# dist1ll/pomcpp

Hardware: NVIDIA B200
Metric: env-steps/sec (higher is better)
Workload: dtype u8/int32

## Files before the change

pomcpp_b200/csrc/pom_batch.cu:

```cuda
#include <cuda_runtime.h>
#include <cstdio>
#include <cstdlib>
#include <cstring>
#include <fstream>
#include <sched.h>
#include <string>
#include <vector>
#include <new>

#include "pom_batch.h"
#include "pom_kernels.cuh"

namespace
{

thread_local std::string g_err;

int fail(int code, const char* what, cudaError_t ce = cudaSuccess)
{
    g_err = what;
    if(ce != cudaSuccess)
    {
        g_err += ": ";
        g_err += cudaGetErrorString(ce);
    }
    return code;
}

struct DevBuf {
    void* p = nullptr;
    ~DevBuf() { if(p) cudaFree(p); }
    cudaError_t alloc(size_t bytes) { return cudaMalloc(&p, bytes); }
    template<typename T> T* as() const { return static_cast<T*>(p); }
};

#define CK(expr) do { cudaError_t ce_ = (expr); if(ce_ != cudaSuccess) return fail(POM_E_CUDA, #expr, ce_); } while(0)

constexpr uint64_t TILE_ALIGN = 256;
constexpr uint64_t XFER_CHUNK = 65536;
constexpr size_t   FLUSH_BYTES = size_t(256) << 20;

}

struct pom_batch {
    int       device = 0;
    uint64_t  n_envs = 0;
    uint64_t  n_alloc = 0;
    uint64_t  env_offset = 0;
    uint32_t  n_templates = 0;
    uint32_t  max_ticks = 0;
    int       tpb = 128;
    int       n_sms = 1;
    int       ws_nw = 20;
    uint32_t  attr_ws = 0;
    uint32_t  walk = 0;
    int       pingpong = 1;
    int       no_spec = 0;
    int       policy_pertick = 1;
    int       obs_fused = 0;
    int       step_kernel = 0;
    bool      teams = false;
    int       policy_view = -1;
    uint8_t*  recs = nullptr;
    uint8_t*  templates = nullptr;
    uint32_t* episodes = nullptr;
    unsigned long long* stats = nullptr;
    uint32_t* moves_buf = nullptr;
    uint8_t*  status_buf = nullptr;
    pom_state* aos_stage = nullptr;
    uint8_t*  st_stage = nullptr;
    uint32_t* bad_count = nullptr;
    uint32_t* fin_counter = nullptr;
    uint32_t* policy = nullptr;
    void*     flush_buf = nullptr;
    uint32_t* idx_buf = nullptr;
    uint64_t  idx_cap = 0;
    cudaEvent_t ev_expand = nullptr;
    cudaStream_t stream = nullptr;
    cudaEvent_t ev[2] = { nullptr, nullptr };
    static constexpr int MAX_CHUNKS = 16;
    cudaStream_t s_h2d = nullptr, s_d2h = nullptr, s_k2 = nullptr;
    cudaEvent_t ev_k2 = nullptr;
    cudaEvent_t ev_in[MAX_CHUNKS] = {}, ev_done[MAX_CHUNKS] = {}, ev_out = nullptr, ev_begin = nullptr;
    std::vector<int32_t> seeds;
    uint64_t  launches = 0;
    bool      forked = false;
    uint32_t  attr_done = 0;

    pomk::BatchParams params() const
    {
        pomk::BatchParams P;
        P.recs = recs; P.n_envs = n_envs; P.env_offset = env_offset; P.templates = templates;
        P.n_templates = n_templates; P.max_ticks = max_ticks;
        P.tmpl_mask = (n_templates & (n_templates - 1u)) == 0u ? n_templates - 1u : 0u; P.episodes = episodes; P.stats = stats;
        P.policy = policy; P.policy_stride = n_alloc;
        return P;
    }
};

namespace
{

int use(const pom_batch* cb, bool join = true)
{
    if(!cb) return fail(POM_E_ARG, "null handle");
    CK(cudaSetDevice(cb->device));
    pom_batch* b = const_cast<pom_batch*>(cb);
    if(join && b->forked)
    {
        CK(cudaEventRecord(b->ev_k2, b->s_k2));
        CK(cudaStreamWaitEvent(b->stream, b->ev_k2, 0));
        b->forked = false;
    }
    return POM_OK;
}

enum { ATTR_STEP = 1, ATTR_ROLLOUT = 2, ATTR_ROLLOUT_POLICY = 4, ATTR_POLICY_MOVES = 8, ATTR_EXPAND = 16, ATTR_OBS = 32, ATTR_ROLLOUT_SPEC = 64, ATTR_OBS_CROPPED = 128 };
constexpr uint32_t attr_bit(uint32_t which, bool teams, bool fog = false) { return (fog ? which << 16 : which) << (teams ? 8 : 0); }

uint32_t policy_view_bits(const pom_batch* b)
{
    return uint32_t(b->policy_view > 15 ? 15 : b->policy_view) << pomk::POLICY_VIEW_SHIFT;
}

template<typename K>
int set_smem(pom_batch* b, uint32_t which, K kernel, uint32_t bytes)
{
    if(b->attr_done & which) return POM_OK;
    CK(cudaFuncSetAttribute(kernel, cudaFuncAttributeMaxDynamicSharedMemorySize, int(bytes)));
    b->attr_done |= which;
    return POM_OK;
}

int ensure_stage(pom_batch* b)
{
    if(!b->aos_stage)
    {
        CK(cudaMalloc(&b->aos_stage, XFER_CHUNK * sizeof(pom_state)));
// ... 23 lines not shown
}

int build_templates_from_seeds(pom_batch* b, int32_t first_seed)
{
    const uint32_t n = b->n_templates;
    if(n > (1u << 24)) return fail(POM_E_ARG, "pom_batch_init: at most 2^24 templates");
    if(int64_t(first_seed) + 16 * int64_t(n) + 4096 > 0x7FFFFFFFll) return fail(POM_E_ARG, "pom_batch_init: first_seed too close to INT_MAX for this many templates");
    uint32_t ncand = uint32_t(n * 2.2) + 64;
    for(int attempt = 0; attempt < 6; attempt++, ncand *= 2)
    {
        DevBuf cand_b, dirty_b, pick_b;
        CK(cand_b.alloc(size_t(ncand) * POM_REC_BYTES));
        CK(dirty_b.alloc(ncand));
        uint8_t* cand = cand_b.as<uint8_t>(); uint8_t* dirty = dirty_b.as<uint8_t>();
        pomk::k_make_templates<<<(ncand + 63) / 64, 64, 0, b->stream>>>(cand, dirty, first_seed, ncand);
        b->launches++;
        CK(cudaGetLastError());
        std::vector<uint8_t> h(ncand);
        CK(cudaMemcpyAsync(h.data(), dirty, ncand, cudaMemcpyDeviceToHost, b->stream));
        CK(cudaStreamSynchronize(b->stream));
        std::vector<uint32_t> idx;
        for(uint32_t i = 0; i < ncand && idx.size() < n; i++) if(!h[i]) idx.push_back(i);
        if(idx.size() == n)
        {
            CK(pick_b.alloc(n * sizeof(uint32_t)));
            uint32_t* pick = pick_b.as<uint32_t>();
            CK(cudaMemcpyAsync(pick, idx.data(), n * sizeof(uint32_t), cudaMemcpyHostToDevice, b->stream));
            const uint64_t words = uint64_t(n) * POM_REC_WORDS;
            pomk::k_gather_records<<<unsigned((words + 255) / 256), 256, 0, b->stream>>>(
                reinterpret_cast<uint32_t*>(b->templates), reinterpret_cast<const uint32_t*>(cand), pick, n, 0);
            b->launches++;
            CK(cudaGetLastError());
            CK(cudaStreamSynchronize(b->stream));
            b->seeds.resize(n);
            for(uint32_t k = 0; k < n; k++) b->seeds[k] = first_seed + int32_t(idx[k]);
            return POM_OK;
        }
    }
    return fail(POM_E_ARG, "could not find enough clean seeds");
}

int pack_into(pom_batch* b, uint8_t* dst_recs, uint64_t first, uint64_t count, const pom_state* states, const uint8_t* status, uint32_t* bad_total)
{
    int rc = ensure_stage(b);
    if(rc) return rc;
    for(uint64_t done = 0; done < count; done += XFER_CHUNK)
    {
        const uint64_t c = count - done < XFER_CHUNK ? count - done : XFER_CHUNK;
        CK(cudaMemcpyAsync(b->aos_stage, states + done, c * sizeof(pom_state), cudaMemcpyHostToDevice, b->stream));
        if(status) CK(cudaMemcpyAsync(b->st_stage, status + done, c, cudaMemcpyHostToDevice, b->stream));
        CK(cudaMemsetAsync(b->bad_count, 0, sizeof(uint32_t), b->stream));
        pomk::k_pack<<<unsigned((c + 127) / 128), 128, 0, b->stream>>>(b->aos_stage, status ? b->st_stage : nullptr, dst_recs, first + done, c, b->bad_count);
        b->launches++;
        CK(cudaGetLastError());
        uint32_t bad = 0;
        CK(cudaMemcpyAsync(&bad, b->bad_count, sizeof(uint32_t), cudaMemcpyDeviceToHost, b->stream));
        CK(cudaStreamSynchronize(b->stream));
        *bad_total += bad;
    }
    return POM_OK;
}

constexpr int WS_NW = 20, WS_NBUF = 24;

template<int NW, bool OBS, bool FREEZE = false, bool SPEC = false, bool TEAMS = false>
int launch_step_ws(pom_batch* b, const pomk::BatchParams& P, const pomk::StepIO& io, uint32_t flags, cudaStream_t on)
{
    typedef pomk::RingScratch<WS_NBUF> R;
    const uint32_t bit = TEAMS ? (1u << (24 + (FREEZE ? 2 : (OBS ? 1 : 0)))) :
                         SPEC ? 2u : (FREEZE ? 1u : (1u << (NW + (OBS ? 1 : 0))));
    if(!(b->attr_ws & bit))
    {
        CK(cudaFuncSetAttribute(pomk::k_step_ws<NW, WS_NBUF, OBS, FREEZE, SPEC, TEAMS>, cudaFuncAttributeMaxDynamicSharedMemorySize, int(R::BYTES)));
        b->attr_ws |= bit;
    }
    const uint64_t n_slices = (P.n_envs + 31) / 32;
    const unsigned grid = unsigned(n_slices < uint64_t(b->n_sms) ? n_slices : uint64_t(b->n_sms));
    pomk::k_step_ws<NW, WS_NBUF, OBS, FREEZE, SPEC, TEAMS><<<grid, (NW + 1) * 32, R::BYTES, on ? on : b->stream>>>(P, io, flags);
    b->launches++;
    CK(cudaGetLastError());
    return POM_OK;
}

int launch_step_io(pom_batch* b, const pomk::BatchParams& P, pomk::StepIO io, uint32_t flags, cudaStream_t on)
{
    io.bulk = (reinterpret_cast<uintptr_t>(io.moves) & 15u) == 0u ? 1u : 0u;
    if(P.n_envs == b->n_envs && b->pingpong) io.reverse = (b->walk++) & 1u;
    if(b->teams)
    {
        if(flags & pomk::STEP_FREEZE_TRUNCATED) return launch_step_ws<WS_NW, false, true, false, true>(b, P, io, flags, on);
        if(io.obs) return launch_step_ws<WS_NW, true, false, false, true>(b, P, io, flags, on);
        return launch_step_ws<WS_NW, false, false, false, true>(b, P, io, flags, on);
    }
    if(flags & pomk::STEP_FREEZE_TRUNCATED) return launch_step_ws<WS_NW, false, true>(b, P, io, flags, on);
    if(b->ws_nw == WS_NW && (flags & ~uint32_t(POM_STEP_OVERLAP)) == uint32_t(POM_STEP_AUTORESET | POM_STEP_COUNT) && io.bulk &&
       !io.status_out && !io.obs && !io.joint && !io.done_bits && !io.fin_env && !b->no_spec)
        return launch_step_ws<WS_NW, false, false, true>(b, P, io, flags, on);
    if(io.obs) return launch_step_ws<WS_NW, true>(b, P, io, flags, on);
    switch(b->ws_nw)
    {
    case 12: return launch_step_ws<12, false>(b, P, io, flags, on);
    case 14: return launch_step_ws<14, false>(b, P, io, flags, on);
    case 16: return launch_step_ws<16, false>(b, P, io, flags, on);
    case 18: return launch_step_ws<18, false>(b, P, io, flags, on);
    case 22: return launch_step_ws<22, false>(b, P, io, flags, on);
    default: return launch_step_ws<WS_NW, false>(b, P, io, flags, on);
    }
}

template<int TPB, bool TEAMS = false>
int launch_step(pom_batch* b, const uint8_t* moves_dev, uint32_t flags, uint8_t* status_dev, uint64_t first = 0, uint64_t count = 0, cudaStream_t on = nullptr,
                bool tile_kernel = false)
{
    pomk::BatchParams P = b->params();
    if(count)
    {
        P.recs += first * POM_REC_BYTES; P.episodes += first; P.env_offset += first; P.n_envs = count;
        moves_dev += 4 * first;
        if(status_dev) status_dev += first;
    }
    if(b->step_kernel == 0 && !tile_kernel)
    {
        pomk::StepIO io{};
        io.moves = moves_dev;
        io.status_out = status_dev;
        return launch_step_io(b, P, io, flags, on);
    }
    { int rc = set_smem(b, attr_bit(ATTR_STEP, TEAMS), pomk::k_step<TPB, TEAMS>, pomk::TileScratch<TPB>::BYTES); if(rc) return rc; }
    const unsigned grid = unsigned((P.n_envs + TPB - 1) / TPB);
    pomk::k_step<TPB, TEAMS><<<grid, TPB, pomk::TileScratch<TPB>::BYTES, on ? on : b->stream>>>(P, reinterpret_cast<const uint32_t*>(moves_dev), flags, status_dev);
    b->launches++;
    CK(cudaGetLastError());
    return POM_OK;
}

template<int TPB, bool TEAMS = false, bool FOG = false>
int launch_rollout(pom_batch* b, uint32_t ticks, uint64_t seed, uint32_t tick0, uint32_t flags, const uint8_t* move_seq = nullptr)
{
    const uint32_t n_actions = (flags & POM_ROLL_HARMLESS) ? 5u : 6u, no_reset = flags & (POM_ROLL_NO_RESET | POM_ROLL_CONTINUE_UNDEFINED);
    const uint32_t mask = (flags >> POM_ROLL_SIMPLE_SHIFT) & 0xFu;
    const unsigned grid = unsigned((b->n_envs + TPB - 1) / TPB);
    if(mask)
    {
        int rc = set_smem(b, attr_bit(ATTR_ROLLOUT_POLICY, TEAMS, FOG), pomk::k_rollout<TPB, true, false, TEAMS, FOG>, pomk::TileScratch<TPB>::BYTES); if(rc) return rc;
        rc = ensure_policy(b); if(rc) return rc;
        pomk::k_rollout<TPB, true, false, TEAMS, FOG><<<grid, TPB, pomk::TileScratch<TPB>::BYTES, b->stream>>>(b->params(), ticks, seed, tick0, n_actions, no_reset,
                                                                                                     FOG ? mask | policy_view_bits(b) : mask, nullptr);
    }
    else if(!TEAMS && n_actions == 6u && no_reset == 0u && !move_seq && !b->no_spec)
    {
        int rc = set_smem(b, ATTR_ROLLOUT_SPEC, pomk::k_rollout<TPB, false, true>, pomk::TileScratch<TPB>::BYTES); if(rc) return rc;
        pomk::k_rollout<TPB, false, true><<<grid, TPB, pomk::TileScratch<TPB>::BYTES, b->stream>>>(b->params(), ticks, seed, tick0, 6u, 0u, 0u, nullptr);
    }
    else
    {
        int rc = set_smem(b, attr_bit(ATTR_ROLLOUT, TEAMS), pomk::k_rollout<TPB, false, false, TEAMS>, pomk::TileScratch<TPB>::BYTES); if(rc) return rc;
        pomk::k_rollout<TPB, false, false, TEAMS><<<grid, TPB, pomk::TileScratch<TPB>::BYTES, b->stream>>>(b->params(), ticks, seed, tick0, n_actions, no_reset, 0u, reinterpret_cast<const uint32_t*>(move_seq));
    }
    b->launches++;
    CK(cudaGetLastError());
    return POM_OK;
}

template<int TPB, bool TEAMS = false, bool FOG = false>
int launch_policy_moves(pom_batch* b, uint8_t* moves_dev, uint64_t seed, uint32_t tick, uint32_t mask, uint32_t gen_actions = 0, uint32_t freeze_truncated = 0)
{
    { int rc = set_smem(b, attr_bit(ATTR_POLICY_MOVES, TEAMS, FOG), pomk::k_policy_moves<TPB, TEAMS, FOG>, pomk::TileScratch<TPB>::BYTES); if(rc) return rc; }
    const unsigned grid = unsigned((b->n_envs + TPB - 1) / TPB);
    pomk::k_policy_moves<TPB, TEAMS, FOG><<<grid, TPB, pomk::TileScratch<TPB>::BYTES, b->stream>>>(b->params(), reinterpret_cast<uint32_t*>(moves_dev), seed, tick,
                                                                                            FOG ? mask | policy_view_bits(b) : mask, gen_actions, freeze_truncated);
    b->launches++;
    CK(cudaGetLastError());
    return POM_OK;
}

template<int TPB>
int launch_observe_planes(pom_batch* b, uint8_t* obs_dev, uint32_t mask, int view, uint32_t cropped_bytes = 0)
{
    const unsigned grid = unsigned((b->n_envs + TPB - 1) / TPB);
    const uint32_t reverse = (b->pingpong && b->walk && ((b->walk - 1u) & 1u) == 0u) ? 1u : 0u;
    if(cropped_bytes)
    {
        int rc = set_smem(b, ATTR_OBS_CROPPED, pomk::k_observe_planes<TPB, true>, pomk::TileScratch<TPB>::BYTES); if(rc) return rc;
        pomk::k_observe_planes<TPB, true><<<grid, TPB, pomk::TileScratch<TPB>::BYTES, b->stream>>>(b->params(), obs_dev, b->n_alloc, mask, view, reverse, cropped_bytes);
    }
    else
    {
        int rc = set_smem(b, ATTR_OBS, pomk::k_observe_planes<TPB, false>, pomk::TileScratch<TPB>::BYTES); if(rc) return rc;
        pomk::k_observe_planes<TPB, false><<<grid, TPB, pomk::TileScratch<TPB>::BYTES, b->stream>>>(b->params(), obs_dev, b->n_alloc, mask, view, reverse, 0u);
    }
    b->launches++;
    CK(cudaGetLastError());
    return POM_OK;
}

template<int TPB, bool TEAMS = false>
int launch_expand(pom_batch* dst, const pom_batch* src, const uint32_t* idx_dev, uint64_t n_children, uint32_t fanout, uint32_t flags)
{
    { int rc = set_smem(dst, attr_bit(ATTR_EXPAND, TEAMS), pomk::k_expand_step<TPB, TEAMS>, pomk::TileScratch<TPB>::BYTES); if(rc) return rc; }
    const unsigned grid = unsigned((n_children + TPB - 1) / TPB);
    pomk::k_expand_step<TPB, TEAMS><<<grid, TPB, pomk::TileScratch<TPB>::BYTES, dst->stream>>>(dst->recs, src->recs, idx_dev, n_children, fanout, flags);
    dst->launches++;
    CK(cudaGetLastError());
    return POM_OK;
}

}

namespace
// ... 15 lines not shown
{
bool local_cpus(int device, cpu_set_t* set)
{
    char bus[32] = {0};
    if(cudaDeviceGetPCIBusId(bus, sizeof(bus), device) != cudaSuccess) { cudaGetLastError(); return false; }
    for(char* c = bus; *c; c++) if(*c >= 'A' && *c <= 'Z') *c = char(*c - 'A' + 'a');
    std::ifstream f(std::string("/sys/bus/pci/devices/") + bus + "/local_cpulist");
    std::string list;
    if(!f || !std::getline(f, list) || list.empty()) return false;
    CPU_ZERO(set);
    int n = 0;
    size_t i = 0;
    while(i < list.size())
    {
        char* end = nullptr;
        const long lo = std::strtol(list.c_str() + i, &end, 10);
        long hi = lo;
        i = size_t(end - list.c_str());
        if(i < list.size() && list[i] == '-') { hi = std::strtol(list.c_str() + i + 1, &end, 10); i = size_t(end - list.c_str()); }
        for(long c = lo; c <= hi && c < CPU_SETSIZE; c++) { CPU_SET(int(c), set); n++; }
        if(i < list.size() && list[i] == ',') i++;
        else if(i < list.size() && (list[i] < '0' || list[i] > '9')) break;
    }
    return n > 0;
}
}

#define POM_DISPATCH(h, fn, ...) \
    do { \
        if((h)->tpb == 32) return fn<32>(__VA_ARGS__); \
        if((h)->tpb == 64) return fn<64>(__VA_ARGS__); \
        if((h)->tpb == 256) return fn<256>(__VA_ARGS__); \
        return fn<128>(__VA_ARGS__); \
    } while(0)
#define POM_DISPATCH_MODE(h, fn, ...) \
    do { \
        if((h)->teams) return fn<128, true>(__VA_ARGS__); \
        POM_DISPATCH(h, fn, __VA_ARGS__); \
    } while(0)
#define POM_DISPATCH_POLICY(h, fn, ...) \
    do { \
        if((h)->policy_view >= 0) \
        { \
            if((h)->teams) return fn<128, true, true>(__VA_ARGS__); \
            return fn<128, false, true>(__VA_ARGS__); \
        } \
        POM_DISPATCH_MODE(h, fn, __VA_ARGS__); \
    } while(0)

extern "C" {

const char* pom_last_error(void) { return g_err.c_str(); }

int pom_device_count(void)
{
    int n = 0;
    if(cudaGetDeviceCount(&n) != cudaSuccess) { cudaGetLastError(); return 0; }
    return n;
}

int pom_batch_init(pom_batch** out, int device, uint64_t n_envs, const pom_init_desc* desc)
{
    if(!out || !desc || n_envs == 0 || desc->n_templates == 0) return fail(POM_E_ARG, "pom_batch_init: bad argument");
    if(n_envs > (uint64_t(1) << 31)) return fail(POM_E_ARG, "pom_batch_init: too many envs for one handle");
    int ndev = 0;
    cudaError_t ce = cudaGetDeviceCount(&ndev);
    if(ce != cudaSuccess || ndev == 0) return fail(POM_E_CUDA, "no CUDA device: the step path has no CPU fallback", ce);
    if(device < 0 || device >= ndev) return fail(POM_E_ARG, "pom_batch_init: no such device");
    CK(cudaSetDevice(device));
    pom_batch* b = new(std::nothrow) pom_batch();
    if(!b) return fail(POM_E_NOMEM, "host allocation failed");
    b->device = device;
    b->n_envs = n_envs;
    b->n_alloc = (n_envs + TILE_ALIGN - 1) / TILE_ALIGN * TILE_ALIGN;
    b->env_offset = desc->env_offset;
    b->n_templates = desc->n_templates;
    b->max_ticks = desc->max_ticks;
    b->teams = (desc->flags & POM_INIT_TEAMS) != 0;
    cudaDeviceGetAttribute(&b->n_sms, cudaDevAttrMultiProcessorCount, device);
    if(b->n_sms < 1) b->n_sms = 1;
    if(const char* e = std::getenv("POM_STEP_KERNEL")) b->step_kernel = std::strcmp(e, "tile") == 0 ? 1 : 0;
    if(const char* e = std::getenv("POM_WS_NW")) b->ws_nw = std::atoi(e);
    if(const char* e = std::getenv("POM_STEP_PINGPONG")) b->pingpong = std::atoi(e) != 0;
    if(const char* e = std::getenv("POM_OBS_FUSED")) b->obs_fused = std::atoi(e) != 0;
    if(const char* e = std::getenv("POM_WS_NOSPEC")) b->no_spec = std::atoi(e) != 0;
    if(const char* e = std::getenv("POM_ROLL_POLICY")) b->policy_pertick = std::strcmp(e, "fused") != 0;
    if(const char* e = std::getenv("POM_TPB"))
    {
        const int t = std::atoi(e);
        if(t == 32 || t == 64 || t == 128 || t == 256) b->tpb = t;
    }
    int rc = POM_OK;
    do {
        if(cudaStreamCreateWithFlags(&b->stream, cudaStreamNonBlocking) != cudaSuccess ||
           cudaEventCreate(&b->ev[0]) != cudaSuccess || cudaEventCreate(&b->ev[1]) != cudaSuccess ||
           cudaStreamCreateWithFlags(&b->s_h2d, cudaStreamNonBlocking) != cudaSuccess ||
           cudaStreamCreateWithFlags(&b->s_d2h, cudaStreamNonBlocking) != cudaSuccess ||
           cudaStreamCreateWithFlags(&b->s_k2, cudaStreamNonBlocking) != cudaSuccess ||
           cudaEventCreateWithFlags(&b->ev_k2, cudaEventDisableTiming) != cudaSuccess ||
           cudaEventCreateWithFlags(&b->ev_out, cudaEventDisableTiming) != cudaSuccess ||
           cudaEventCreateWithFlags(&b->ev_begin, cudaEventDisableTiming) != cudaSuccess)
        { rc = fail(POM_E_CUDA, "stream/event creation failed", cudaGetLastError()); break; }
        if(cudaMalloc(&b->recs, b->n_alloc * POM_REC_BYTES) != cudaSuccess ||
           cudaMalloc(&b->templates, size_t(b->n_templates) * POM_REC_BYTES) != cudaSuccess ||
           cudaMalloc(&b->episodes, b->n_alloc * sizeof(uint32_t)) != cudaSuccess ||
           cudaMalloc(&b->stats, POM_STATS_WORDS * sizeof(unsigned long long)) != cudaSuccess ||
           cudaMalloc(&b->moves_buf, b->n_alloc * 4) != cudaSuccess ||
           cudaMalloc(&b->status_buf, b->n_alloc) != cudaSuccess)
        { rc = fail(POM_E_NOMEM, "device allocation failed", cudaGetLastError()); break; }
        if(cudaMemsetAsync(b->recs, 0, b->n_alloc * POM_REC_BYTES, b->stream) != cudaSuccess ||
           cudaMemsetAsync(b->episodes, 0, b->n_alloc * sizeof(uint32_t), b->stream) != cudaSuccess ||
           cudaMemsetAsync(b->stats, 0, POM_STATS_WORDS * sizeof(unsigned long long), b->stream) != cudaSuccess)
        { rc = fail(POM_E_CUDA, "memset failed", cudaGetLastError()); break; }
        if(desc->host_templates)
        {
            uint32_t bad = 0;
            rc = pack_into(b, b->templates, 0, b->n_templates, desc->host_templates, nullptr, &bad);
            if(rc) break;
            if(bad) { rc = fail(POM_E_STATE, "a host template cannot be represented in the packed record"); break; }
        }
        else
        {
            rc = build_templates_from_seeds(b, desc->first_seed);
            if(rc) break;
        }
        if(!(desc->flags & POM_INIT_EMPTY))
        {
            rc = fill_from_templates(b);
            if(rc) break;
        }
        if(cudaStreamSynchronize(b->stream) != cudaSuccess) { rc = fail(POM_E_CUDA, "init sync failed", cudaGetLastError()); break; }
    } while(0);
    if(rc) { pom_batch_destroy(b); return rc; }
    *out = b;
    return POM_OK;
}

int pom_batch_destroy(pom_batch* b)
{
    if(!b) return POM_OK;
    cudaSetDevice(b->device);
    if(b->s_k2) cudaStreamSynchronize(b->s_k2);
    if(b->stream) cudaStreamSynchronize(b->stream);
    cudaFree(b->recs); cudaFree(b->templates); cudaFree(b->episodes); cudaFree(b->stats);
    cudaFree(b->moves_buf); cudaFree(b->status_buf); cudaFree(b->aos_stage); cudaFree(b->st_stage);
    cudaFree(b->bad_count); cudaFree(b->flush_buf); cudaFree(b->idx_buf); if(b->ev_expand) cudaEventDestroy(b->ev_expand); cudaFree(b->policy); cudaFree(b->fin_counter);
    if(b->ev[0]) cudaEventDestroy(b->ev[0]);
    if(b->ev[1]) cudaEventDestroy(b->ev[1]);
    for(int i = 0; i < pom_batch::MAX_CHUNKS; i++) { if(b->ev_in[i]) cudaEventDestroy(b->ev_in[i]); if(b->ev_done[i]) cudaEventDestroy(b->ev_done[i]); }
    if(b->ev_out) cudaEventDestroy(b->ev_out);
    if(b->ev_begin) cudaEventDestroy(b->ev_begin);
    if(b->s_h2d) cudaStreamDestroy(b->s_h2d);
    if(b->s_d2h) cudaStreamDestroy(b->s_d2h);
    if(b->s_k2) cudaStreamDestroy(b->s_k2);
    if(b->ev_k2) cudaEventDestroy(b->ev_k2);
    if(b->stream) cudaStreamDestroy(b->stream);
    delete b;
    return POM_OK;
}

int pom_batch_sync(pom_batch* b)
{
    int rc = use(b); if(rc) return rc;
    CK(cudaStreamSynchronize(b->stream));
    return POM_OK;
}
// ... 26 lines not shown
        CK(cudaStreamSynchronize(b->stream));
    }
    return POM_OK;
}

int pom_batch_observe(pom_batch* b, uint64_t first, uint64_t count, int agent, int view, pom_state* states, uint8_t* status)
{
    int rc = use(b); if(rc) return rc;
    if(!states) return fail(POM_E_ARG, "pom_batch_observe: null output");
    if(agent < 0 || agent > 3 || view < 0) return fail(POM_E_ARG, "pom_batch_observe: agent must be 0..3 and view >= 0");
    if(first > b->n_envs || count > b->n_envs - first) return fail(POM_E_RANGE, "pom_batch_observe: range outside the batch");
    rc = ensure_stage(b); if(rc) return rc;
    for(uint64_t done = 0; done < count; done += XFER_CHUNK)
    {
        const uint64_t c = count - done < XFER_CHUNK ? count - done : XFER_CHUNK;
        pomk::k_observe<<<unsigned((c + 127) / 128), 128, 0, b->stream>>>(b->recs, b->aos_stage, b->st_stage, first + done, c, agent, view);
        b->launches++;
        CK(cudaGetLastError());
        CK(cudaMemcpyAsync(states + done, b->aos_stage, c * sizeof(pom_state), cudaMemcpyDeviceToHost, b->stream));
        if(status) CK(cudaMemcpyAsync(status + done, b->st_stage, c, cudaMemcpyDeviceToHost, b->stream));
        CK(cudaStreamSynchronize(b->stream));
    }
    return POM_OK;
}

uint64_t pom_batch_obs_stride(const pom_batch* b) { return b ? b->n_alloc : 0; }

int pom_batch_observe_planes(pom_batch* b, uint8_t* obs_dev, uint32_t agent_mask, int view)
{
    int rc = use(b); if(rc) return rc;
    if(!obs_dev) return fail(POM_E_ARG, "pom_batch_observe_planes: null output");
    if(agent_mask == 0 || agent_mask > 0xFu || view < 0) return fail(POM_E_ARG, "pom_batch_observe_planes: agent_mask must be 1..15 and view >= 0");
    POM_DISPATCH(b, launch_observe_planes, b, obs_dev, agent_mask, view);
}

int pom_device_copy(int device, void* dst, const void* src, uint64_t bytes)
{
    if(!dst || !src) return fail(POM_E_ARG, "pom_device_copy: null pointer");
    CK(cudaSetDevice(device));
    CK(cudaMemcpy(dst, src, bytes, cudaMemcpyDefault));
    return POM_OK;
}

int pom_batch_reset(pom_batch* b)
{
    int rc = use(b); if(rc) return rc;
    CK(cudaMemsetAsync(b->episodes, 0, b->n_alloc * sizeof(uint32_t), b->stream));
    CK(cudaMemsetAsync(b->stats, 0, POM_STATS_WORDS * sizeof(unsigned long long), b->stream));
    if(b->policy) CK(cudaMemsetAsync(b->policy, 0, 9 * b->n_alloc * sizeof(uint32_t), b->stream));
    return fill_from_templates(b);
}

int pom_batch_templates(pom_batch* b, pom_state* out, int32_t* seeds_out)
{
    int rc = use(b); if(rc) return rc;
    if(!out) return fail(POM_E_ARG, "pom_batch_templates: null output");
    rc = ensure_stage(b); if(rc) return rc;
    for(uint64_t done = 0; done < b->n_templates; done += XFER_CHUNK)
    {
        const uint64_t c = b->n_templates - done < XFER_CHUNK ? b->n_templates - done : XFER_CHUNK;
        pomk::k_unpack<<<unsigned((c + 127) / 128), 128, 0, b->stream>>>(b->templates, b->aos_stage, b->st_stage, done, c);
        b->launches++;
        CK(cudaGetLastError());
        CK(cudaMemcpyAsync(out + done, b->aos_stage, c * sizeof(pom_state), cudaMemcpyDeviceToHost, b->stream));
        CK(cudaStreamSynchronize(b->stream));
    }
    if(seeds_out)
    {
        for(uint32_t k = 0; k < b->n_templates; k++) seeds_out[k] = k < b->seeds.size() ? b->seeds[k] : 0;
    }
    return POM_OK;
}

int pom_batch_step(pom_batch* b, const uint8_t* moves_dev, uint32_t flags)
{
    const bool overlap = (flags & POM_STEP_OVERLAP) && b && b->n_envs >= (uint64_t(1) << 18);
    int rc = use(b, !overlap); if(rc) return rc;
    if(!moves_dev) return fail(POM_E_ARG, "pom_batch_step: null moves");
    if(!overlap) POM_DISPATCH_MODE(b, launch_step, b, moves_dev, flags, nullptr);
    static int parts = -1;
    if(parts < 0) { const char* e = std::getenv("POM_STEP_PARTS"); parts = e ? std::atoi(e) : 2; if(parts < 2 || parts > 16) parts = 2; }
    const uint64_t per = ((b->n_envs + parts - 1) / parts + 1023) / 1024 * 1024;
    const bool tile_parts = b->n_envs <= (uint64_t(1) << 19) && !b->no_spec;
    CK(cudaEventRecord(b->ev_begin, b->stream));
    CK(cudaStreamWaitEvent(b->s_k2, b->ev_begin, 0));
    int c = 0;
    for(uint64_t first = 0; first < b->n_envs; first += per, c++)
    {
        const uint64_t count = first + per <= b->n_envs ? per : b->n_envs - first;
        rc = [&]() -> int { POM_DISPATCH_MODE(b, launch_step, b, moves_dev, flags, nullptr, first, count, (c & 1) ? b->s_k2 : b->stream, tile_parts); }();
        if(rc) return rc;
    }
    b->forked = true;
    return POM_OK;
}

static int enqueue_step_pipeline(pom_batch* b, const uint8_t* moves_host, uint8_t* status_host, uint32_t flags, int chunks, uint64_t per)
{
    const uint64_t n = b->n_envs;
    CK(cudaEventRecord(b->ev_begin, b->stream));
    CK(cudaStreamWaitEvent(b->s_h2d, b->ev_begin, 0));
    if(chunks > 1) CK(cudaStreamWaitEvent(b->s_k2, b->ev_begin, 0));
    for(int c = 0; c < chunks; c++)
    {
        const uint64_t first = uint64_t(c) * per, count = (first + per <= n) ? per : n - first;
        cudaStream_t compute = (c & 1) ? b->s_k2 : b->stream;
        CK(cudaMemcpyAsync(reinterpret_cast<uint8_t*>(b->moves_buf) + 4 * first, moves_host + 4 * first, 4 * count, cudaMemcpyHostToDevice, b->s_h2d));
        CK(cudaEventRecord(b->ev_in[c], b->s_h2d));
        CK(cudaStreamWaitEvent(compute, b->ev_in[c], 0));
        const int rc = [&]() -> int { POM_DISPATCH_MODE(b, launch_step, b, reinterpret_cast<const uint8_t*>(b->moves_buf), flags,
                                                   status_host ? b->status_buf : nullptr, first, count, compute); }();
        if(rc) return rc;
        if(status_host)
        {
            CK(cudaEventRecord(b->ev_done[c], compute));
            CK(cudaStreamWaitEvent(b->s_d2h, b->ev_done[c], 0));
            CK(cudaMemcpyAsync(status_host + first, b->status_buf + first, count, cudaMemcpyDeviceToHost, b->s_d2h));
        }
    }
    if(chunks > 1)
    {
        CK(cudaEventRecord(b->ev_k2, b->s_k2));
        CK(cudaStreamWaitEvent(b->stream, b->ev_k2, 0));
    }
    if(status_host)
    {
        CK(cudaEventRecord(b->ev_out, b->s_d2h));
        CK(cudaStreamWaitEvent(b->stream, b->ev_out, 0));
    }
    return POM_OK;
}

static int launch_step_zero_copy(pom_batch* b, const uint8_t* moves_host, uint8_t* status_host, uint32_t flags)
{
    void* mdev = nullptr; void* sdev = nullptr;
    bool ok = cudaHostGetDevicePointer(&mdev, const_cast<uint8_t*>(moves_host), 0) == cudaSuccess;
    if(ok && status_host) ok = cudaHostGetDevicePointer(&sdev, status_host, 0) == cudaSuccess;
    if(!ok) { cudaGetLastError(); return 1; }
    return [&]() -> int { POM_DISPATCH_MODE(b, launch_step, b, static_cast<const uint8_t*>(mdev), flags, static_cast<uint8_t*>(sdev)); }();
}

int pom_batch_step_host_async(pom_batch* b, const uint8_t* moves_host, uint8_t* status_host, uint32_t flags)
{
    int rc = use(b); if(rc) return rc;
    if(!moves_host) return fail(POM_E_ARG, "pom_batch_step_host_async: null moves");
    rc = launch_step_zero_copy(b, moves_host, status_host, flags);
    if(rc == 1) return fail(POM_E_ARG, "pom_batch_step_host_async: the buffers must be page-locked, device-mapped memory (pom_host_alloc)");
    return rc;
}

int pom_batch_step_host(pom_batch* b, const uint8_t* moves_host, uint8_t* status_host, uint32_t flags)
{
    int rc = use(b); if(rc) return rc;
    if(!moves_host) return fail(POM_E_ARG, "pom_batch_step_host: null moves");
    const uint64_t n = b->n_envs;
    static int zerocopy = -1;
    if(zerocopy < 0) { const char* e = std::getenv("POM_ZEROCOPY"); zerocopy = e ? std::atoi(e) : 1; }
    if(zerocopy)
    {
        rc = launch_step_zero_copy(b, moves_host, status_host, flags);
        if(rc < 0) return rc;
        if(rc == 0)
        {
            CK(cudaStreamSynchronize(b->stream));
            return POM_OK;
        }
    }
    static int want = -1;
    if(want < 0) { const char* e = std::getenv("POM_CHUNKS"); want = e ? std::atoi(e) : 6; if(want < 1 || want > pom_batch::MAX_CHUNKS) want = 6; }
    int chunks = n >= (uint64_t(1) << 18) ? want : 1;
    const uint64_t per = ((n + chunks - 1) / chunks + 1023) / 1024 * 1024;
    chunks = int((n + per - 1) / per);
    for(int c = 0; c < chunks; c++)
// ... 447 lines not shown
```

pomcpp_b200/csrc/pom_kernels.cuh:

```cuda
#ifndef POM_KERNELS_CUH_
#define POM_KERNELS_CUH_

#include <cuda_runtime.h>
#include <stdint.h>
#include "pom_core.cuh"
#include "pom_policy.cuh"
#include "pom_batch.h"

namespace pomk
{

constexpr uint32_t STEP_FREEZE_TRUNCATED = 0x40000000u;

enum { ST_STEPS = 0, ST_EPISODES = 1, ST_WIN0 = 2, ST_DRAWS = 6, ST_TRUNC = 7, ST_SUMLEN = 8, ST_INVALID = 9 };

struct BatchParams {
    uint8_t*            recs;
    uint64_t            n_envs;
    uint64_t            env_offset;
    const uint8_t*      templates;
    uint32_t            n_templates;
    uint32_t            tmpl_mask;
    uint32_t            max_ticks;
    uint32_t*           episodes;
    unsigned long long* stats;
    uint32_t*           policy;
    uint64_t            policy_stride;
};

__device__ __forceinline__ uint32_t smem_u32(const void* p) { return uint32_t(__cvta_generic_to_shared(p)); }

__device__ __forceinline__ void mbar_init(uint64_t* bar, uint32_t count)
{
    asm volatile("mbarrier.init.shared::cta.b64 [%0], %1;" :: "r"(smem_u32(bar)), "r"(count));
}
__device__ __forceinline__ void fence_barrier_init()
{
    asm volatile("fence.mbarrier_init.release.cluster;" ::: "memory");
}
__device__ __forceinline__ void fence_proxy_async()
{
    asm volatile("fence.proxy.async.shared::cta;" ::: "memory");
}
__device__ __forceinline__ void mbar_expect_tx(uint64_t* bar, uint32_t bytes)
{
    asm volatile("mbarrier.arrive.expect_tx.shared::cta.b64 _, [%0], %1;" :: "r"(smem_u32(bar)), "r"(bytes) : "memory");
}
__device__ __forceinline__ void mbar_arrive(uint64_t* bar)
{
    asm volatile("mbarrier.arrive.shared::cta.b64 _, [%0];" :: "r"(smem_u32(bar)) : "memory");
}
__device__ __forceinline__ void mbar_wait(uint64_t* bar, uint32_t parity)
{
    asm volatile(
        "{\n"
        ".reg .pred p;\n"
        "WAIT_LOOP:\n"
        "mbarrier.try_wait.parity.shared::cta.b64 p, [%0], %1;\n"
        "@p bra WAIT_DONE;\n"
        "bra WAIT_LOOP;\n"
        "WAIT_DONE:\n"
        "}\n" :: "r"(smem_u32(bar)), "r"(parity) : "memory");
}
__device__ __forceinline__ void bulk_g2s(void* smem_dst, const void* gmem_src, uint32_t bytes, uint64_t* bar)
{
    asm volatile("cp.async.bulk.shared::cluster.global.mbarrier::complete_tx::bytes [%0], [%1], %2, [%3];"
                 :: "r"(smem_u32(smem_dst)), "l"(gmem_src), "r"(bytes), "r"(smem_u32(bar)) : "memory");
}
__device__ __forceinline__ void bulk_s2g(void* gmem_dst, const void* smem_src, uint32_t bytes)
{
    asm volatile("cp.async.bulk.global.shared::cta.bulk_group [%0], [%1], %2;"
                 :: "l"(gmem_dst), "r"(smem_u32(smem_src)), "r"(bytes) : "memory");
    asm volatile("cp.async.bulk.commit_group;" ::: "memory");
}
__device__ __forceinline__ void bulk_wait_read_all()
{
    asm volatile("cp.async.bulk.wait_group.read 0;" ::: "memory");
}

__device__ __forceinline__ void warp_add(unsigned long long* dst, uint32_t v)
{
    const uint32_t s = __reduce_add_sync(0xFFFFFFFFu, v);
    if((threadIdx.x & 31u) == 0u && s) atomicAdd(dst, (unsigned long long)s);
}

struct EpisodeAcc {
    uint32_t fin_draw = 0u;
    uint32_t trunc_abort = 0u;
    uint32_t win01 = 0u, win23 = 0u;
    uint32_t len = 0u;
    uint32_t steps = 0u;
    uint32_t pending = 0u;
};

__device__ __forceinline__ void acc_add(EpisodeAcc& A, bool fin, uint32_t status, uint32_t len)
{
    if(!fin) return;
    const bool done = (status & POM_STATUS_DONE) != 0u;
    const bool draw = done && (status & POM_STATUS_DRAW);
    const bool trunc = !done && (status & POM_STATUS_TRUNCATED);
    const uint32_t w = (status & POM_STATUS_WINNER_MASK) >> POM_STATUS_WINNER_SHIFT;
    A.fin_draw += 1u + (draw ? 0x10000u : 0u);
    A.trunc_abort += (trunc ? 1u : 0u) + ((!done && !trunc) ? 0x10000u : 0u);
    if(done && !draw)
    {
        const uint32_t inc = (w & 1u) ? 0x10000u : 1u;
        if(w & 2u) A.win23 += inc; else A.win01 += inc;
    }
    A.len += len;
    A.pending++;
}

__device__ __forceinline__ void acc_flush(unsigned long long* stats, EpisodeAcc& A, bool count_steps)
{
    const uint32_t lane = threadIdx.x & 31u;
    if(__reduce_or_sync(0xFFFFFFFFu, A.pending))
    {
        const uint32_t v[9] = { A.fin_draw & 0xFFFFu, A.win01 & 0xFFFFu, A.win01 >> 16, A.win23 & 0xFFFFu, A.win23 >> 16,
                                A.fin_draw >> 16, A.trunc_abort & 0xFFFFu, A.len, A.trunc_abort >> 16 };
#pragma unroll
        for(int k = 0; k < 9; k++)
        {
            const uint32_t sum = __reduce_add_sync(0xFFFFFFFFu, v[k]);
            if(lane == 0u && sum) atomicAdd(stats + 1 + k, (unsigned long long)sum);
        }
    }
    if(count_steps)
    {
        const uint32_t sum = __reduce_add_sync(0xFFFFFFFFu, A.steps);
        if(lane == 0u && sum) atomicAdd(stats + ST_STEPS, (unsigned long long)sum);
    }
    A = EpisodeAcc();
}

__device__ __forceinline__ void cp_async_4(void* smem_dst, const void* gmem_src)
{
    asm volatile("cp.async.ca.shared.global [%0], [%1], 4;" :: "r"(smem_u32(smem_dst)), "l"(gmem_src) : "memory");
}
__device__ __forceinline__ void cp_async_wait_all()
{
    asm volatile("cp.async.wait_all;" ::: "memory");
}

__device__ __forceinline__ uint32_t finish_and_reset(uint8_t* warp_recs, uint8_t* rec, const BatchParams& P, uint64_t env, bool active, bool do_reset,
                                                 uint32_t& ep_now, EpisodeAcc& acc)
{
    uint32_t st = active ? rec[R_STATUS] : 0u;
    const uint32_t len = active ? *reinterpret_cast<const uint16_t*>(rec + R_TIME) : 0u;
    if(active && !(st & POM_STATUS_DONE) && P.max_ticks && len >= P.max_ticks) st |= POM_STATUS_TRUNCATED;
    const bool fin = active && (st & (POM_STATUS_DONE | POM_STATUS_TRUNCATED | POM_STATUS_INVALID)) != 0u;
    uint32_t pending = __ballot_sync(0xFFFFFFFFu, fin);
    if(pending == 0u) return st;
    acc_add(acc, fin, st, len);
    if(!do_reset)
    {
        if(fin) rec[R_STATUS] = uint8_t(st);
        return st;
// ... 147 lines not shown
{
    const uint32_t lane = threadIdx.x & 31u, quad = lane >> 2;
    const int part = int(lane & 3u);
#pragma unroll 1
    for(uint32_t m = 0; m < 4u; m++)
    {
        const uint32_t e = quad + 8u * m;
        const bool valid = e < n_valid;
        const uint8_t* r = sslice + e * POM_REC_BYTES;
        uint8_t* out = out0 + size_t(e) * POM_OBS_BYTES;
        pomcore::ObsWindow W{};
        uint32_t lit = 0u;
        if(valid)
        {
            W = pomcore::obs_window(r, agent, view);
            lit = pomcore::observe_part_chunks(r, agent, W, out, part);
        }
        lit |= __shfl_xor_sync(FULL_WARP, lit, 1);
        lit |= __shfl_xor_sync(FULL_WARP, lit, 2);
        __syncwarp();
        if(valid) pomcore::observe_part_patches(r, W, out, part, lit);
    }
}

template<int TPB> struct TileScratch {
    static constexpr uint32_t OFF_BAR = TPB * POM_REC_BYTES;
    static constexpr uint32_t OFF_LIST = OFF_BAR + 64;
    static constexpr uint32_t BYTES = OFF_LIST + 8 * (TPB / 32);
};

template<int TPB, bool TEAMS = false>
__global__ void __launch_bounds__(TPB) k_step(BatchParams P, const uint32_t* __restrict__ moves, uint32_t flags, uint8_t* __restrict__ status_out)
{
    extern __shared__ __align__(128) uint8_t smem[];
    const uint64_t env = uint64_t(blockIdx.x) * TPB + threadIdx.x;
    const bool active = env < P.n_envs;
    const bool raw = (flags & POM_STEP_RAW) != 0u;

    constexpr uint32_t SLICE_BYTES = 32 * POM_REC_BYTES;
    const uint32_t warp = threadIdx.x >> 5, lane = threadIdx.x & 31u;
    uint64_t* bar = reinterpret_cast<uint64_t*>(smem + TileScratch<TPB>::OFF_BAR) + warp;
    uint8_t* sslice = smem + warp * SLICE_BYTES;
    uint8_t* gslice = P.recs + (size_t(blockIdx.x) * TPB + warp * 32u) * POM_REC_BYTES;
    if(lane == 0)
    {
        mbar_init(bar, 1);
        fence_barrier_init();
        mbar_expect_tx(bar, SLICE_BYTES);
        bulk_g2s(sslice, gslice, SLICE_BYTES, bar);
    }
    const uint32_t m = active ? __ldg(moves + env) : 0u;
    uint32_t ep_now = (active && (flags & POM_STEP_AUTORESET)) ? P.episodes[env] : 0u;
    __syncwarp();
    mbar_wait(bar, 0);

    uint8_t* rec = sslice + lane * POM_REC_BYTES;
    const bool stepped = active && !(rec[R_STATUS] & (raw ? POM_STATUS_INVALID : (POM_STATUS_DONE | POM_STATUS_INVALID)));
    warp_tick<TEAMS>(sslice, rec, m, stepped, raw, smem + TileScratch<TPB>::OFF_LIST + 8u * warp,
                     (flags & POM_STEP_CONTINUE_UNDEFINED) ? pomcore::F_INVALID_MASK_CONTINUE : pomcore::F_INVALID_MASK);
    EpisodeAcc acc;
    acc.steps = stepped ? 1u : 0u;
    uint32_t st_end = active ? rec[R_STATUS] : 0u;
    if(flags & POM_STEP_AUTORESET)
    {
        const uint32_t st = finish_and_reset(sslice, rec, P, env, active && stepped, true, ep_now, acc);
        if(active && stepped) st_end = st;
    }
    acc_flush(P.stats, acc, (flags & POM_STEP_COUNT) != 0u);
    if(status_out && active) status_out[env] = uint8_t(st_end);
    fence_proxy_async();
    __syncwarp();
    if(lane == 0)
    {
        bulk_s2g(gslice, sslice, SLICE_BYTES);
        bulk_wait_read_all();
    }
}

struct StepIO {
    const void* moves;
    uint32_t    joint;
    uint32_t    bulk;
    uint32_t    reverse;
    uint8_t*    status_out;
    uint32_t*   done_bits;
    uint32_t*   fin_env;
    uint8_t*    fin_status;
    uint32_t*   fin_counter;
    uint32_t*   fin_count_out;
    uint32_t    fin_capacity;
    uint8_t*    obs;
    uint64_t    obs_stride;
    uint32_t    obs_mask;
    int         obs_view;
};

__device__ __forceinline__ uint32_t moves_of_joint(uint32_t j)
{
    const uint32_t a0 = j % 6u, r1 = j / 6u, a1 = r1 % 6u, r2 = r1 / 6u, a2 = r2 % 6u, a3 = (r2 / 6u) % 6u;
    return a0 | (a1 << 8) | (a2 << 16) | (a3 << 24);
}

template<int NBUF> struct RingScratch {
    static constexpr uint32_t SLICE_BYTES = 32 * POM_REC_BYTES;
    static constexpr uint32_t SLOT = SLICE_BYTES + 128 + 16;
    static constexpr uint32_t OFF_FULL = NBUF * SLOT;
    static constexpr uint32_t MAIL = 256;
    static constexpr uint32_t OFF_MAIL = OFF_FULL + 8 * NBUF;
    static constexpr uint32_t OFF_TICKET = OFF_MAIL + 4 * MAIL;
    static constexpr uint32_t FIN_CAP = 480;
    static constexpr uint32_t OFF_FIN = OFF_TICKET + 16;
    static constexpr uint32_t OFF_FIN_ENV = OFF_FIN + 16;
    static constexpr uint32_t OFF_FIN_ST = OFF_FIN_ENV + 4 * FIN_CAP;
    static constexpr uint32_t BYTES = OFF_FIN_ST + FIN_CAP;
};

template<int NW, int NBUF, bool OBS, bool FREEZE, bool SPEC = false, bool TEAMS = false>
__global__ void __launch_bounds__((NW + 1) * 32, 1) k_step_ws(BatchParams P, StepIO io_in, uint32_t flags_in)
{
    const uint32_t flags = SPEC ? uint32_t(POM_STEP_AUTORESET | POM_STEP_COUNT) : flags_in;
    StepIO io = io_in;
    if(SPEC)
    {
        io.joint = 0u; io.bulk = 1u; io.status_out = nullptr; io.obs = nullptr; io.done_bits = nullptr; io.fin_env = nullptr;
    }
    const uint32_t* __restrict__ moves = static_cast<const uint32_t*>(io.moves);
    const uint16_t* __restrict__ joint = static_cast<const uint16_t*>(io.moves);
    uint8_t* __restrict__ status_out = io.status_out;
    const uint32_t moves_bulk = io.bulk;
    const uint32_t mv_bytes = io.joint ? 64u : 128u;
    extern __shared__ __align__(128) uint8_t smem[];
    typedef RingScratch<NBUF> R;
    uint64_t* full = reinterpret_cast<uint64_t*>(smem + R::OFF_FULL);
    volatile uint32_t* mail = reinterpret_cast<volatile uint32_t*>(smem + R::OFF_MAIL);
    uint32_t* ticket = reinterpret_cast<uint32_t*>(smem + R::OFF_TICKET);
    uint32_t* free_mask = ticket + 2;
    const uint32_t warp = threadIdx.x >> 5, lane = threadIdx.x & 31u;
    const uint64_t n_slices = (P.n_envs + 31u) / 32u;
    const uint32_t T = blockIdx.x < n_slices ? uint32_t((n_slices - blockIdx.x + gridDim.x - 1u) / gridDim.x) : 0u;
    if(threadIdx.x == 0)
    {
        for(int b = 0; b < NBUF; b++) mbar_init(full + b, 1);
        ticket[0] = 0u;
        ticket[1] = 0u;
        *free_mask = (NBUF >= 32) ? 0xFFFFFFFFu : ((1u << NBUF) - 1u);
        reinterpret_cast<uint32_t*>(smem + R::OFF_FIN)[0] = 0u;
        reinterpret_cast<uint32_t*>(smem + R::OFF_FIN)[1] = 0xFFFFFFFFu;
        fence_barrier_init();
    }
    for(uint32_t i = threadIdx.x; i < R::MAIL; i += blockDim.x) mail[i] = 0u;
    __syncthreads();

    if(warp == NW)
    {
        if(lane != 0) return;
        uint32_t parity = 0u;
        for(uint32_t t = 0; t < T; t++)
        {
            uint32_t fm;
            while((fm = *reinterpret_cast<volatile uint32_t*>(free_mask)) == 0u) __nanosleep(40);
            const uint32_t b = uint32_t(__ffs(int(fm))) - 1u;
            atomicAnd(free_mask, ~(1u << b));
            const uint64_t s0 = blockIdx.x + uint64_t(t) * gridDim.x;
            const uint64_t s = io.reverse ? n_slices - 1u - s0 : s0;
            const bool whole = (s + 1u) * 32u <= P.n_envs;
            const uint32_t mbytes = (moves_bulk && whole) ? mv_bytes : 0u;
            mbar_expect_tx(full + b, R::SLICE_BYTES + mbytes);
            bulk_g2s(smem + b * R::SLOT, P.recs + s * R::SLICE_BYTES, R::SLICE_BYTES, full + b);
            if(mbytes) bulk_g2s(smem + b * R::SLOT + R::SLICE_BYTES, static_cast<const uint8_t*>(io.moves) + s * mv_bytes, mbytes, full + b);
            mail[t % R::MAIL] = ((t + 1u) << 8) | (b << 1) | ((parity >> b) & 1u);
            parity ^= 1u << b;
        }
        return;
    }

    const bool raw = (flags & POM_STEP_RAW) != 0u;
    EpisodeAcc acc;
    for(;;)
    {
        uint32_t t = 0u;
        if(lane == 0) t = atomicAdd(ticket, 1u);
        t = __shfl_sync(FULL_WARP, t, 0);
        if(t >= T) break;
        const uint64_t s0 = blockIdx.x + uint64_t(t) * gridDim.x;
        const uint64_t s = io.reverse ? n_slices - 1u - s0 : s0;
        const uint64_t env = s * 32u + lane;
        const bool active = env < P.n_envs;
        const bool whole = (s + 1u) * 32u <= P.n_envs;
        uint32_t m = 0u;
        if(!(moves_bulk && whole) && active) m = io.joint ? uint32_t(__ldg(joint + env)) : __ldg(moves + env);
        uint32_t ep_now = (active && (flags & POM_STEP_AUTORESET)) ? P.episodes[env] : 0u;
        uint32_t v;
        while(((v = mail[t % R::MAIL]) >> 8) != t + 1u) __nanosleep(20);
        const uint32_t b = (v >> 1) & 31u;
        uint8_t* sslice = smem + b * R::SLOT;
        mbar_wait(full + b, v & 1u);
        if(moves_bulk && whole)
            m = io.joint ? uint32_t(reinterpret_cast<const uint16_t*>(sslice + R::SLICE_BYTES)[lane])
                         : reinterpret_cast<const uint32_t*>(sslice + R::SLICE_BYTES)[lane];
        if(io.joint) m = moves_of_joint(m);

        uint8_t* rec = sslice + lane * POM_REC_BYTES;
        const bool stepped = active && !(rec[R_STATUS] & ((raw ? POM_STATUS_INVALID : (POM_STATUS_DONE | POM_STATUS_INVALID)) |
                                                          (FREEZE ? POM_STATUS_TRUNCATED : 0)));
        warp_tick<TEAMS>(sslice, rec, m, stepped, raw, sslice + R::SLICE_BYTES + 128u,
                         (flags & POM_STEP_CONTINUE_UNDEFINED) ? pomcore::F_INVALID_MASK_CONTINUE : pomcore::F_INVALID_MASK);
        acc.steps += stepped ? 1u : 0u;
        uint32_t st_end = active ? rec[R_STATUS] : 0u;
        if(flags & POM_STEP_AUTORESET)
        {
            const uint32_t st = finish_and_reset(sslice, rec, P, env, active && stepped, true, ep_now, acc);
            if(active && stepped) st_end = st;
        }
        if(status_out && active) status_out[env] = uint8_t(st_end);
        if(io.done_bits || io.fin_env)
        {
            const bool ended = active && stepped && (st_end & (POM_STATUS_DONE | POM_STATUS_TRUNCATED | POM_STATUS_INVALID)) != 0u;
            const uint32_t em = __ballot_sync(FULL_WARP, ended);
            if(io.done_bits && lane == 0) io.done_bits[s] = em;
            if(io.fin_env && em)
            {
                uint32_t* fin = reinterpret_cast<uint32_t*>(smem + R::OFF_FIN);
                const uint32_t k = uint32_t(__popc(em));
                uint32_t pos = 0u;
                if(lane == 0) pos = atomicAdd(fin, k);
                pos = __shfl_sync(FULL_WARP, pos, 0);
                const uint32_t mine = uint32_t(__popc(em & ((1u << lane) - 1u)));
                if(pos + k <= R::FIN_CAP)
                {
                    if(ended)
                    {
                        reinterpret_cast<uint32_t*>(smem + R::OFF_FIN_ENV)[pos + mine] = uint32_t(env);
                        smem[R::OFF_FIN_ST + pos + mine] = uint8_t(st_end);
                    }
                }
                else
                {
                    if(lane == 0) { atomicMin(fin + 1, pos); pos = atomicAdd(io.fin_counter, k); }
                    pos = __shfl_sync(FULL_WARP, pos, 0) + mine;
                    if(ended && pos < io.fin_capacity)
                    {
                        io.fin_env[pos] = uint32_t(env);
                        io.fin_status[pos] = uint8_t(st_end);
                    }
                }
            }
        }
        fence_proxy_async();
        __syncwarp();
        if(lane == 0) bulk_s2g(P.recs + s * R::SLICE_BYTES, sslice, R::SLICE_BYTES);
        if(OBS && io.obs)
        {
            const uint32_t n_valid = whole ? 32u : uint32_t(P.n_envs - s * 32u);
            uint32_t k = 0u;
            for(int a = 0; a < 4; a++)
            {
                if(!((io.obs_mask >> a) & 1u)) continue;
                warp_observe_slice(sslice, a, io.obs_view, io.obs + (uint64_t(k) * io.obs_stride + s * 32u) * POM_OBS_BYTES, n_valid);
                k++;
            }
        }
        __syncwarp();
        if(lane == 0)
        {
            bulk_wait_read_all();
            __threadfence_block();
            atomicOr(free_mask, 1u << b);
        }
        __syncwarp();
    }
    acc_flush(P.stats, acc, (flags & POM_STEP_COUNT) != 0u);
    if(io.fin_env)
    {
        __threadfence_block();
        uint32_t* warps_done = ticket + 1;
        bool last = false;
        if(lane == 0) last = atomicAdd(warps_done, 1u) == uint32_t(NW - 1);
        last = __shfl_sync(FULL_WARP, last ? 1 : 0, 0) != 0;
        if(last)
        {
            __threadfence_block();
            const volatile uint32_t* fin = reinterpret_cast<const volatile uint32_t*>(smem + R::OFF_FIN);
            const uint32_t k = fin[1] != 0xFFFFFFFFu ? fin[1] : fin[0];
            unsigned long long old = 0ull;
            if(lane == 0) old = atomicAdd(reinterpret_cast<unsigned long long*>(io.fin_counter), (1ull << 32) | k);
            old = __shfl_sync(FULL_WARP, old, 0);
            const uint32_t base = uint32_t(old);
            for(uint32_t i = lane; i < k; i += 32u)
            {
                if(base + i < io.fin_capacity)
                {
                    io.fin_env[base + i] = reinterpret_cast<const uint32_t*>(smem + R::OFF_FIN_ENV)[i];
                    io.fin_status[base + i] = smem[R::OFF_FIN_ST + i];
                }
            }
            if(lane == 0 && uint32_t(old >> 32) == gridDim.x - 1u)
            {
                const uint32_t count = base + k;
                *io.fin_count_out = count < io.fin_capacity ? count : io.fin_capacity;
                *reinterpret_cast<volatile unsigned long long*>(io.fin_counter) = 0ull;
            }
        }
    }
}

struct GlobalAgentStore {
    uint32_t* base;
    uint64_t  stride;
    __device__ __forceinline__ pompolicy::SimpleSt load(int a) const
    {
        pompolicy::SimpleSt s;
        s.w0 = base[uint64_t(2 * a) * stride];
        s.w1 = base[uint64_t(2 * a + 1) * stride];
        return s;
    }
    __device__ __forceinline__ void store(int a, const pompolicy::SimpleSt& v)
    {
        base[uint64_t(2 * a) * stride] = v.w0;
        base[uint64_t(2 * a + 1) * stride] = v.w1;
    }
    __device__ __forceinline__ void clear(uint32_t episode)
    {
#pragma unroll
        for(int k = 0; k < 8; k++) base[uint64_t(k) * stride] = 0u;
        base[8 * stride] = episode;
    }
    __device__ __forceinline__ void claim(uint32_t episode)
    {
        if(base[8 * stride] != episode) clear(episode);
    }
};

constexpr uint32_t POLICY_VIEW_SHIFT = 8;
// ... 359 lines not shown
```

Measured before the change: 10.06 billion.

## Keep last tickets of each step part L2-resident with cache-hint bulk copies

In the split multi-stream step path, all parts now share the same walk direction, and the bulk loads and stores of env records carry L2 cache-policy hints. Earlier tickets use evict_first, and the last tickets (about 16 MB by default, set by an env var) use evict_normal. The goal is for the slices touched last by one step to still sit in L2 when the next step, walking the opposite way, reads them first, which cuts HBM traffic. It only applies when the state exceeds L2 but is at most four times L2, and it adds policy creation instructions on the producer and consumer paths.

```diff
diff --git a/pomcpp_b200/csrc/pom_batch.cu b/pomcpp_b200/csrc/pom_batch.cu
--- a/pomcpp_b200/csrc/pom_batch.cu
+++ b/pomcpp_b200/csrc/pom_batch.cu
@@ -39,6 +39,7 @@
 constexpr uint64_t TILE_ALIGN = 256;
 constexpr uint64_t XFER_CHUNK = 65536;
 constexpr size_t   FLUSH_BYTES = size_t(256) << 20;
+constexpr uint64_t L2_KEEP_MB = 16;
 
 }
 
@@ -54,6 +55,8 @@
     int       ws_nw = 20;
     uint32_t  attr_ws = 0;
     uint32_t  walk = 0;
+    uint64_t  l2_keep_bytes = uint64_t(L2_KEEP_MB) << 20;
+    uint64_t  l2_bytes = 0;
     int       pingpong = 1;
     int       no_spec = 0;
     int       policy_pertick = 1;
@@ -243,10 +246,24 @@
     return POM_OK;
 }
 
-int launch_step_io(pom_batch* b, const pomk::BatchParams& P, pomk::StepIO io, uint32_t flags, cudaStream_t on)
+uint32_t l2_keep(const pom_batch* b, uint64_t n_envs)
+{
+    if(!b->l2_keep_bytes || b->n_envs * POM_REC_BYTES <= b->l2_bytes) return 0u;
+    const uint64_t n_slices = (n_envs + 31) / 32, grid = n_slices < uint64_t(b->n_sms) ? n_slices : uint64_t(b->n_sms);
+    const uint64_t per_ticket = grid * 32 * POM_REC_BYTES, tickets = (n_slices + grid - 1) / grid;
+    const uint64_t keep = (b->l2_keep_bytes + per_ticket - 1) / per_ticket;
+    return uint32_t(keep < tickets ? keep : tickets);
+}
+
+int launch_step_io(pom_batch* b, const pomk::BatchParams& P, pomk::StepIO io, uint32_t flags, cudaStream_t on, int part = -1)
 {
     io.bulk = (reinterpret_cast<uintptr_t>(io.moves) & 15u) == 0u ? 1u : 0u;
-    if(P.n_envs == b->n_envs && b->pingpong) io.reverse = (b->walk++) & 1u;
+    if(part < 0 && P.n_envs == b->n_envs && b->pingpong) io.reverse = (b->walk++) & 1u;
+    if(part >= 0)
+    {
+        io.reverse = (b->walk - 1u) & 1u;
+        io.keep = l2_keep(b, P.n_envs);
+    }
     if(b->teams)
     {
         if(flags & pomk::STEP_FREEZE_TRUNCATED) return launch_step_ws<WS_NW, false, true, false, true>(b, P, io, flags, on);
@@ -271,7 +288,7 @@
 
 template<int TPB, bool TEAMS = false>
 int launch_step(pom_batch* b, const uint8_t* moves_dev, uint32_t flags, uint8_t* status_dev, uint64_t first = 0, uint64_t count = 0, cudaStream_t on = nullptr,
-                bool tile_kernel = false)
+                bool tile_kernel = false, int part = -1)
 {
     pomk::BatchParams P = b->params();
     if(count)
@@ -285,7 +302,7 @@
         pomk::StepIO io{};
         io.moves = moves_dev;
         io.status_out = status_dev;
-        return launch_step_io(b, P, io, flags, on);
+        return launch_step_io(b, P, io, flags, on, part);
     }
     { int rc = set_smem(b, attr_bit(ATTR_STEP, TEAMS), pomk::k_step<TPB, TEAMS>, pomk::TileScratch<TPB>::BYTES); if(rc) return rc; }
     const unsigned grid = unsigned((P.n_envs + TPB - 1) / TPB);
@@ -467,6 +484,8 @@
     if(const char* e = std::getenv("POM_STEP_KERNEL")) b->step_kernel = std::strcmp(e, "tile") == 0 ? 1 : 0;
     if(const char* e = std::getenv("POM_WS_NW")) b->ws_nw = std::atoi(e);
     if(const char* e = std::getenv("POM_STEP_PINGPONG")) b->pingpong = std::atoi(e) != 0;
+    if(const char* e = std::getenv("POM_STEP_L2_KEEP_MB")) { const uint64_t mb = std::strtoull(e, nullptr, 10); b->l2_keep_bytes = (mb < 65536 ? mb : 65536) << 20; }
+    { int l2 = 0; cudaDeviceGetAttribute(&l2, cudaDevAttrL2CacheSize, device); b->l2_bytes = uint64_t(l2 > 0 ? l2 : 0); }
     if(const char* e = std::getenv("POM_OBS_FUSED")) b->obs_fused = std::atoi(e) != 0;
     if(const char* e = std::getenv("POM_WS_NOSPEC")) b->no_spec = std::atoi(e) != 0;
     if(const char* e = std::getenv("POM_ROLL_POLICY")) b->policy_pertick = std::strcmp(e, "fused") != 0;
@@ -659,13 +678,15 @@
     if(parts < 0) { const char* e = std::getenv("POM_STEP_PARTS"); parts = e ? std::atoi(e) : 2; if(parts < 2 || parts > 16) parts = 2; }
     const uint64_t per = ((b->n_envs + parts - 1) / parts + 1023) / 1024 * 1024;
     const bool tile_parts = b->n_envs <= (uint64_t(1) << 19) && !b->no_spec;
+    const bool part_walk = !tile_parts && b->pingpong && b->n_envs * POM_REC_BYTES <= 4 * b->l2_bytes;
+    if(part_walk) b->walk++;
     CK(cudaEventRecord(b->ev_begin, b->stream));
     CK(cudaStreamWaitEvent(b->s_k2, b->ev_begin, 0));
     int c = 0;
     for(uint64_t first = 0; first < b->n_envs; first += per, c++)
     {
         const uint64_t count = first + per <= b->n_envs ? per : b->n_envs - first;
-        rc = [&]() -> int { POM_DISPATCH_MODE(b, launch_step, b, moves_dev, flags, nullptr, first, count, (c & 1) ? b->s_k2 : b->stream, tile_parts); }();
+        rc = [&]() -> int { POM_DISPATCH_MODE(b, launch_step, b, moves_dev, flags, nullptr, first, count, (c & 1) ? b->s_k2 : b->stream, tile_parts, part_walk ? c : -1); }();
         if(rc) return rc;
     }
     b->forked = true;
diff --git a/pomcpp_b200/csrc/pom_kernels.cuh b/pomcpp_b200/csrc/pom_kernels.cuh
--- a/pomcpp_b200/csrc/pom_kernels.cuh
+++ b/pomcpp_b200/csrc/pom_kernels.cuh
@@ -73,6 +73,29 @@
                  :: "l"(gmem_dst), "r"(smem_u32(smem_src)), "r"(bytes) : "memory");
     asm volatile("cp.async.bulk.commit_group;" ::: "memory");
 }
+__device__ __forceinline__ void bulk_g2s_hint(void* smem_dst, const void* gmem_src, uint32_t bytes, uint64_t* bar, uint64_t pol)
+{
+    asm volatile("cp.async.bulk.shared::cluster.global.mbarrier::complete_tx::bytes.L2::cache_hint [%0], [%1], %2, [%3], %4;"
+                 :: "r"(smem_u32(smem_dst)), "l"(gmem_src), "r"(bytes), "r"(smem_u32(bar)), "l"(pol) : "memory");
+}
+__device__ __forceinline__ void bulk_s2g_hint(void* gmem_dst, const void* smem_src, uint32_t bytes, uint64_t pol)
+{
+    asm volatile("cp.async.bulk.global.shared::cta.bulk_group.L2::cache_hint [%0], [%1], %2, %3;"
+                 :: "l"(gmem_dst), "r"(smem_u32(smem_src)), "r"(bytes), "l"(pol) : "memory");
+    asm volatile("cp.async.bulk.commit_group;" ::: "memory");
+}
+__device__ __forceinline__ uint64_t l2_evict_first()
+{
+    uint64_t pol;
+    asm volatile("createpolicy.fractional.L2::evict_first.b64 %0, 1.0;" : "=l"(pol));
+    return pol;
+}
+__device__ __forceinline__ uint64_t l2_evict_normal()
+{
+    uint64_t pol;
+    asm volatile("createpolicy.fractional.L2::evict_normal.b64 %0, 1.0;" : "=l"(pol));
+    return pol;
+}
 __device__ __forceinline__ void bulk_wait_read_all()
 {
     asm volatile("cp.async.bulk.wait_group.read 0;" ::: "memory");
@@ -386,6 +409,7 @@
     uint32_t    joint;
     uint32_t    bulk;
     uint32_t    reverse;
+    uint32_t    keep;
     uint8_t*    status_out;
     uint32_t*   done_bits;
     uint32_t*   fin_env;
@@ -470,8 +494,17 @@
             const bool whole = (s + 1u) * 32u <= P.n_envs;
             const uint32_t mbytes = (moves_bulk && whole) ? mv_bytes : 0u;
             mbar_expect_tx(full + b, R::SLICE_BYTES + mbytes);
-            bulk_g2s(smem + b * R::SLOT, P.recs + s * R::SLICE_BYTES, R::SLICE_BYTES, full + b);
-            if(mbytes) bulk_g2s(smem + b * R::SLOT + R::SLICE_BYTES, static_cast<const uint8_t*>(io.moves) + s * mv_bytes, mbytes, full + b);
+            if(SPEC && io.keep)
+            {
+                const uint64_t first = l2_evict_first(), normal = l2_evict_normal();
+                bulk_g2s_hint(smem + b * R::SLOT, P.recs + s * R::SLICE_BYTES, R::SLICE_BYTES, full + b, t + io.keep >= T ? normal : first);
+                if(mbytes) bulk_g2s_hint(smem + b * R::SLOT + R::SLICE_BYTES, static_cast<const uint8_t*>(io.moves) + s * mv_bytes, mbytes, full + b, first);
+            }
+            else
+            {
+                bulk_g2s(smem + b * R::SLOT, P.recs + s * R::SLICE_BYTES, R::SLICE_BYTES, full + b);
+                if(mbytes) bulk_g2s(smem + b * R::SLOT + R::SLICE_BYTES, static_cast<const uint8_t*>(io.moves) + s * mv_bytes, mbytes, full + b);
+            }
             mail[t % R::MAIL] = ((t + 1u) << 8) | (b << 1) | ((parity >> b) & 1u);
             parity ^= 1u << b;
         }
@@ -552,7 +585,11 @@
         }
         fence_proxy_async();
         __syncwarp();
-        if(lane == 0) bulk_s2g(P.recs + s * R::SLICE_BYTES, sslice, R::SLICE_BYTES);
+        if(lane == 0)
+        {
+            if(SPEC && io.keep) bulk_s2g_hint(P.recs + s * R::SLICE_BYTES, sslice, R::SLICE_BYTES, t + io.keep >= T ? l2_evict_normal() : l2_evict_first());
+            else bulk_s2g(P.recs + s * R::SLICE_BYTES, sslice, R::SLICE_BYTES);
+        }
         if(OBS && io.obs)
         {
             const uint32_t n_valid = whole ? 32u : uint32_t(P.n_envs - s * 32u);
```

After: 10.31 billion (median of 6 runs). 2.5% higher.
